# yurimjeon1892/EFGH

Measured on AMD Instinct MI355X. Metric: frame-pairs/sec EFGHNet fwd+bwd (384x1280 RGB + 64x2048 range), whole job, higher is better.
Workload: dtype f32; 1 GPU; BASELINE.json configs[2]: EFGHNet fwd+bwd with efghloss + gradient all-reduce + fused Adam, synthetic 384x1280 RGB + 131072-point sweep, batch=8 per GPU, random-init weights; global_batch=8, points=131072, parallelism=dp1

## Files before the change

efgh_amd/csrc/wgrad.hip:

```cpp
#include "common.h"

namespace {

typedef float f32x16 __attribute__((ext_vector_type(16)));
constexpr int TK = 128, TM = 32, LD = 128;

struct WArgs {
    const float *A; int64_t lda;
    int C, T, K;
    unsigned magicC;
    int Hin, Win, Hv, Wv, sh, sw;
    unsigned long long dhpack, dwpack;
    int Ho, Wo, osh, osw, oh0, ow0;
    const int *table;
    const float *G; int64_t ldg;
    int N;
    int tld;
    long long M; int mchunk;
    float *dW;
    long long zstride;
    unsigned kt, nt;
    long long bsA, bsG, bsD;
};

// ... 64 lines not shown
    }
    float4 rg[NGQ], ra[4];
    auto load_step = [&](long long ms) {
        if (TN != 128) {
#pragma unroll
            for (int q = 0; q < NGQ; ++q) {
                long long m = ms + gr0 + GRS * q;
                float4 g = make_float4(0.f, 0.f, 0.f, 0.f);
                if (m < mend && nin) g = *reinterpret_cast<const float4 *>(MODE == 1 ? git[q].g : p.G + m * p.ldg + n0 + gc4);
                rg[q] = g;
                if (MODE == 1) advance(git[q], n0 + gc4);
            }
        }
#pragma unroll
        for (int q = 0; q < 4; ++q) {
            long long m = ms + r0 + 8 * q;
            float4 g = make_float4(0.f, 0.f, 0.f, 0.f), a = g;
            if (m < mend) {
                if (MODE == 1) {
                    if (TN == 128 && nin) g = *reinterpret_cast<const float4 *>(rit[q].g);
                    if (kin && rit[q].rowok && (unsigned)(rit[q].j * p.sw + dw) < (unsigned)p.Win)
                        a = *reinterpret_cast<const float4 *>(rit[q].a);
                } else {
                    long long arow = -1;
                    if (MODE == 0) arow = m;
                    else if (kin) arow = p.table[m * (MODE == 4 ? p.tld : 16) + t];
                    if (TN == 128 && nin) g = *reinterpret_cast<const float4 *>(p.G + m * p.ldg + n0 + c4);
                    if (kin && arow >= 0) a = *reinterpret_cast<const float4 *>(p.A + arow * p.lda + c);
                }
            }
            if (TN == 128) rg[q] = g;
            ra[q] = a;
            if (MODE == 1) advance(rit[q], n0 + c4);
        }
    };

    f32x16 acc[2][TJ];
#pragma unroll
    for (int i = 0; i < 2; ++i)
#pragma unroll
        for (int j = 0; j < TJ; ++j)
#pragma unroll
            for (int r = 0; r < 16; ++r) acc[i][j][r] = 0.f;

    load_step(mbeg);
    for (long long ms = mbeg; ms < mend; ms += TM) {
#pragma unroll
        for (int q = 0; q < 4; ++q)
            *reinterpret_cast<float4 *>(&As[(r0 + 8 * q) * LD + c4]) = ra[q];
#pragma unroll
        for (int q = 0; q < NGQ; ++q)
            *reinterpret_cast<float4 *>(&Gs[(gr0 + GRS * q) * TN + gc4]) = rg[q];
        __syncthreads();
        if (ms + TM < mend) load_step(ms + TM);
#pragma unroll
        for (int mm = 0; mm < TM / 2; ++mm) {
            float g[2], a[TJ];
#pragma unroll
            for (int i = 0; i < 2; ++i) g[i] = Gs[(mm * 2 + lh) * TN + (wn * 2 + i) * 32 + l31];
#pragma unroll
            for (int j = 0; j < TJ; ++j) a[j] = As[(mm * 2 + lh) * LD + (wk * TJ + j) * 32 + l31];
#pragma unroll
            for (int i = 0; i < 2; ++i)
#pragma unroll
                for (int j = 0; j < TJ; ++j)
                    acc[i][j] = __builtin_amdgcn_mfma_f32_32x32x2f32(g[i], a[j], acc[i][j], 0, 0, 0);
        }
        __syncthreads();
    }
#pragma unroll
    for (int i = 0; i < 2; ++i)
#pragma unroll
        for (int j = 0; j < TJ; ++j) {
            const int k = k0 + (wk * TJ + j) * 32 + l31;
            if (k >= p.K) continue;
#pragma unroll
            for (int r = 0; r < 16; ++r) {
                const int n = n0 + (wn * 2 + i) * 32 + (r & 3) + 8 * (r >> 2) + 4 * lh;
                if (n < p.N) p.dW[(long long)n * p.K + k] = acc[i][j][r];
            }
        }
}

typedef efgh_wgrad_out_desc FoldUnpackArgs;

template <bool UNPACK>
__global__ void __launch_bounds__(256) k_fold_splits(const float4 *part, int zs, long long total4, float4 *dst, const FoldUnpackArgs u) {
    __shared__ float4 red[256];
    const int e = threadIdx.x & 15, zl = threadIdx.x >> 4;
    const long long i = (long long)blockIdx.x * 16 + e;
    float4 a = make_float4(0.f, 0.f, 0.f, 0.f), b = a;
    if (i < total4) {
        int z = zl;
        for (; z + 16 < zs; z += 32) {
            const float4 u = part[(long long)z * total4 + i], v = part[(long long)(z + 16) * total4 + i];
            a.x += u.x; a.y += u.y; a.z += u.z; a.w += u.w;
            b.x += v.x; b.y += v.y; b.z += v.z; b.w += v.w;
        }
        if (z < zs) { const float4 u = part[(long long)z * total4 + i]; a.x += u.x; a.y += u.y; a.z += u.z; a.w += u.w; }
        a.x += b.x; a.y += b.y; a.z += b.z; a.w += b.w;
    }
    red[threadIdx.x] = a;
    __syncthreads();
    for (int h = 8; h; h >>= 1) {
        if (zl < h) {
            const float4 o = red[threadIdx.x + h * 16];
            float4 m = red[threadIdx.x];
            m.x += o.x; m.y += o.y; m.z += o.z; m.w += o.w;
            red[threadIdx.x] = m;
        }
        __syncthreads();
    }
    if (zl == 0 && i < total4) {
        if (!UNPACK) { dst[i] = red[e]; return; }
        const float4 v4 = red[e];
        const float v[4] = {v4.x, v4.y, v4.z, v4.w};
        const long long idx = 4 * i;
        const int c0 = (int)(idx % u.Cp); const long long r = idx / u.Cp;
        const int t = (int)(r % u.T), n = (int)(r / u.T);
        if (n >= u.N) return;
        int ti = 0;
#pragma unroll
        for (int q = 0; q < 16; ++q) if (q == t) ti = u.taps[q];
#pragma unroll
        for (int q = 0; q < 4; ++q) {
            if (c0 + q >= u.C) continue;
            float *d = &u.W[n * u.sn + (c0 + q) * u.sc + ti * u.st];
            *d = u.accumulate ? *d + v[q] : v[q];
        }
    }
}

__global__ void k_unpack_weight(const float *__restrict__ Wp, float *__restrict__ W, int N, int T, int C,
                                int Cp, long long sn, long long sc, long long st, const int4 taps0,
                                const int4 taps1, const int4 taps2, const int4 taps3, int accumulate) {
    const int tp[16] = {taps0.x, taps0.y, taps0.z, taps0.w, taps1.x, taps1.y, taps1.z, taps1.w,
                        taps2.x, taps2.y, taps2.z, taps2.w, taps3.x, taps3.y, taps3.z, taps3.w};
    long long total = (long long)N * T * C;
    for (long long i = (long long)blockIdx.x * blockDim.x + threadIdx.x; i < total;
         i += (long long)gridDim.x * blockDim.x) {
        int c = (int)(i % C); long long r = i / C;
        int t = (int)(r % T); int n = (int)(r / T);
        int ti = 0;
#pragma unroll
        for (int q = 0; q < 16; ++q) if (q == t) ti = tp[q];
        float v = Wp[((long long)n * T + t) * Cp + c];
        float *dst = &W[n * sn + c * sc + ti * st];
        *dst = accumulate ? *dst + v : v;
    }
}

__global__ void __launch_bounds__(256)
k_table_scatter_add(const float *__restrict__ src, const int *__restrict__ table, long long M, int T, int C,
                    float *__restrict__ dst) {
    const int c4n = C >> 2;
    long long total = M * T * c4n;
    for (long long i = (long long)blockIdx.x * 256 + threadIdx.x; i < total; i += (long long)gridDim.x * 256) {
        int cq = (int)(i % c4n); long long r = i / c4n;
        int t = (int)(r % T); long long m = r / T;
        int row = table[m * 16 + t];
        if (row < 0) continue;
        float4 v = *reinterpret_cast<const float4 *>(src + (m * T + t) * C + cq * 4);
        float *d = dst + (long long)row * C + cq * 4;
        atomicAdd(d + 0, v.x); atomicAdd(d + 1, v.y); atomicAdd(d + 2, v.z); atomicAdd(d + 3, v.w);
    }
}

}

bool efgh_launch_fold_splits(const float *part, int zs, long long total, float *dst, hipStream_t st, const efgh_wgrad_out_desc *out) {
    const long long total4 = total / 4;
    const unsigned grid = (unsigned)((total4 + 15) / 16);
    if (out && out->W && out->T >= 1 && out->T <= 16 && out->Cp >= out->C && out->Cp % 4 == 0) {
        const long long row = (long long)out->T * out->Cp;
        if (total % row == 0 && total / row >= out->N && total / row < out->N + 4) {
            k_fold_splits<true><<<grid, 256, 0, st>>>((const float4 *)part, zs, total4, (float4 *)dst, *out);
            return true;
        }
    }
    FoldUnpackArgs none = {};
    k_fold_splits<false><<<grid, 256, 0, st>>>((const float4 *)part, zs, total4, (float4 *)dst, none);
    return false;
}

static int gather_wgrad_impl(const efgh_gemm_desc *d, const float *G, int64_t ldg, float *dWp, float *workspace, int nbatch,
                             int64_t bsG, int64_t bsD, const efgh_wgrad_out_desc *out, void *stream_, int tld = 0);


static long long wgrad_chunks(const efgh_gemm_desc *d, int nbatch, long long *chunk_out) {
    const int K = d->T * d->C;
    const int TN = d->N <= 64 ? 64 : 128;
    const long long kt = (K + TK - 1) / TK, nt = (d->N + TN - 1) / TN;
    static const int occ128[3] = {efgh_wg_per_cu((const void *)k_gather_wgrad<0, 128>, 256, 0), efgh_wg_per_cu((const void *)k_gather_wgrad<1, 128>, 256, 0),
                                  efgh_wg_per_cu((const void *)k_gather_wgrad<2, 128>, 256, 0)};
    static const int occ64[3] = {efgh_wg_per_cu((const void *)k_gather_wgrad<0, 64>, 256, 0), efgh_wg_per_cu((const void *)k_gather_wgrad<1, 64>, 256, 0),
                                 efgh_wg_per_cu((const void *)k_gather_wgrad<2, 64>, 256, 0)};
    const int mode = d->mode >= 0 && d->mode <= 2 ? d->mode : 0;
    return efgh_round_chunks(d->M, kt * nt * nbatch, TN == 128 ? occ128[mode] : occ64[mode], TM, 256, (double)nbatch * d->N * K, chunk_out);
}

extern "C" int64_t efgh_gather_wgrad_workspace(const efgh_gemm_desc *d) {
    if (!d || d->C <= 0 || d->T < 1 || d->N < 1 || d->M < 1) return 0;
    const int nbatch = d->nbatch > 1 ? d->nbatch : 1;
    const long long zs = wgrad_chunks(d, nbatch, nullptr);
    return zs > 1 ? zs * nbatch * (int64_t)d->N * d->T * d->C : 0;
}

extern "C" int efgh_gather_wgrad(const efgh_gemm_desc *d, const float *G, int64_t ldg, float *dWp, float *workspace,
                                 const efgh_wgrad_out_desc *out, void *stream_) {
    return gather_wgrad_impl(d, G, ldg, dWp, workspace, 1, 0, 0, out, stream_);
}

extern "C" int efgh_gather_wgrad_batched(const efgh_gemm_desc *d, const float *G, int64_t ldg, int64_t batch_stride_g,
                                         float *dWp, int64_t batch_stride_dw, float *workspace, void *stream_) {
    EFGH_CHECK_ARG(d && d->mode == 0 && d->nbatch >= 1 && d->nbatch <= 65535);
    EFGH_CHECK_ARG(d->batch_stride_a % 4 == 0 && batch_stride_g % 4 == 0 && batch_stride_dw == (int64_t)d->N * d->C);
    return gather_wgrad_impl(d, G, ldg, dWp, workspace, d->nbatch, batch_stride_g, batch_stride_dw, nullptr, stream_);
}

static int gather_wgrad_impl(const efgh_gemm_desc *d, const float *G, int64_t ldg, float *dWp, float *workspace, int nbatch,
                             int64_t bsG, int64_t bsD, const efgh_wgrad_out_desc *out, void *stream_, int tld) {
    hipStream_t st = (hipStream_t)stream_;
    EFGH_CHECK_ARG(d && d->A && G && dWp);
    EFGH_CHECK_ARG(d->C > 0 && d->C % 4 == 0 && d->T >= 1 && (d->T <= 16 || tld > 0) && d->N >= 1 && d->M >= 1);
    EFGH_CHECK_ARG(tld == 0 || (d->mode == 2 && d->table != nullptr && tld >= d->T && nbatch == 1 && !out));
    EFGH_CHECK_ARG(d->lda % 4 == 0 && ldg % 4 == 0 && d->N % 4 == 0);
    EFGH_CHECK_ARG((((uintptr_t)d->A) & 15) == 0 && (((uintptr_t)G) & 15) == 0 && (((uintptr_t)dWp) & 15) == 0);
    EFGH_CHECK_ARG((int64_t)d->T * d->C < 65536 && d->mode >= 0 && d->mode <= 2);
    WArgs a;
    a.A = d->A; a.lda = d->lda; a.C = d->C; a.T = d->T; a.K = d->T * d->C;
    a.magicC = (unsigned)((0x100000000ULL + d->C - 1) / d->C);
    a.Hin = d->Hin; a.Win = d->Win; a.Hv = d->Hv; a.Wv = d->Wv; a.sh = d->sh; a.sw = d->sw;
    a.dhpack = 0; a.dwpack = 0;
    for (int t = 0; t < 16; ++t) {
        int dh = t < d->T ? d->dh[t] : 0, dw = t < d->T ? d->dw[t] : 0;
        a.dhpack |= (unsigned long long)((dh + 8) & 15) << (4 * t);
        a.dwpack |= (unsigned long long)((dw + 8) & 15) << (4 * t);
    }
    a.Ho = d->Ho; a.Wo = d->Wo; a.osh = d->osh; a.osw = d->osw; a.oh0 = d->oh0; a.ow0 = d->ow0;
    a.table = d->table; a.G = G; a.ldg = ldg; a.N = d->N; a.M = d->M;
    a.bsA = nbatch > 1 ? d->batch_stride_a : 0; a.bsG = bsG; a.bsD = bsD; a.tld = tld;
    if (d->mode == 1) EFGH_CHECK_ARG(d->M == (int64_t)d->B * d->Hv * d->Wv && d->osh >= 1 && d->osw >= 1);
    if (d->mode == 2) EFGH_CHECK_ARG(d->table != nullptr);
    const int TN = a.N <= 64 ? 64 : 128;
    const int kt = (a.K + TK - 1) / TK, nt = (a.N + TN - 1) / TN;
    long long chunk = 0;
    const long long zs = wgrad_chunks(d, nbatch, &chunk);
    a.mchunk = (int)chunk;
    EFGH_CHECK_ARG(zs * kt * nt < 0x7fffffffLL);
    a.kt = (unsigned)kt; a.nt = (unsigned)nt;
    const long long plane = (long long)nbatch * a.N * a.K;
    EFGH_CHECK_ARG(zs == 1 || (workspace && (((uintptr_t)workspace) & 15) == 0));
    a.dW = zs > 1 ? workspace : dWp;
    a.zstride = zs > 1 ? plane : 0;
    const dim3 grid((unsigned)(zs * kt * nt), (unsigned)nbatch);
    if (tld > 0) {
        if (TN == 128) k_gather_wgrad<4, 128><<<grid, 256, 0, st>>>(a);
        else k_gather_wgrad<4, 64><<<grid, 256, 0, st>>>(a);
    } else if (TN == 128) {
        if (d->mode == 0) k_gather_wgrad<0, 128><<<grid, 256, 0, st>>>(a);
        else if (d->mode == 1) k_gather_wgrad<1, 128><<<grid, 256, 0, st>>>(a);
        else k_gather_wgrad<2, 128><<<grid, 256, 0, st>>>(a);
    } else {
        if (d->mode == 0) k_gather_wgrad<0, 64><<<grid, 256, 0, st>>>(a);
        else if (d->mode == 1) k_gather_wgrad<1, 64><<<grid, 256, 0, st>>>(a);
        else k_gather_wgrad<2, 64><<<grid, 256, 0, st>>>(a);
    }
    bool wrote = false;
    if (zs > 1) wrote = efgh_launch_fold_splits(workspace, (int)zs, plane, dWp, st, nbatch == 1 ? out : nullptr);
    EFGH_CHECK_LAUNCH();
    return wrote ? EFGH_WROTE_OUT : EFGH_OK;
}

extern "C" int efgh_blur_r_wgrad(const efgh_gemm_desc *d, int32_t ld, const float *G, int64_t ldg, float *dWp, float *workspace,
                                 void *stream_) {
    EFGH_CHECK_ARG(ld > 0);
    const int rc = gather_wgrad_impl(d, G, ldg, dWp, workspace, 1, 0, 0, nullptr, stream_, ld);
    return rc == EFGH_WROTE_OUT ? EFGH_OK : rc;
}

extern "C" int efgh_unpack_weight(const float *Wp, float *W, int32_t N, int32_t T, int32_t C, int32_t Cp,
                                  int64_t sn, int64_t sc, int64_t stt, const int32_t *tapidx, int32_t accumulate,
                                  void *stream_) {
    EFGH_CHECK_ARG(Wp && W && N > 0 && T > 0 && T <= 16 && C > 0 && Cp >= C);
    int tp[16];
    for (int t = 0; t < 16; ++t) tp[t] = (tapidx && t < T) ? tapidx[t] : (t < T ? t : 0);
    long long total = (long long)N * T * C;
    int grid = (int)((total + 255) / 256);
    if (grid > 8192) grid = 8192;
    k_unpack_weight<<<grid, 256, 0, (hipStream_t)stream_>>>(Wp, W, N, T, C, Cp, sn, sc, stt,
                                                           make_int4(tp[0], tp[1], tp[2], tp[3]),
                                                           make_int4(tp[4], tp[5], tp[6], tp[7]),
                                                           make_int4(tp[8], tp[9], tp[10], tp[11]),
                                                           make_int4(tp[12], tp[13], tp[14], tp[15]), accumulate);
    EFGH_CHECK_LAUNCH();
    return EFGH_OK;
}

extern "C" int efgh_table_scatter_add(const float *src, const int32_t *table, int64_t M, int32_t T, int32_t C,
                                      float *dst, void *stream_) {
    EFGH_CHECK_ARG(src && table && dst && M > 0 && T > 0 && T <= 16 && C % 4 == 0);
    long long total = M * T * (C / 4);
    long long g = (total + 255) / 256;
    k_table_scatter_add<<<(int)(g > 16384 ? 16384 : g), 256, 0, (hipStream_t)stream_>>>(src, table, M, T, C, dst);
    EFGH_CHECK_LAUNCH();
    return EFGH_OK;
}

extern "C" int efgh_debug_occupancy(char *out, int32_t cap) {
    EFGH_CHECK_ARG(out && cap > 64);
    snprintf(out, cap, "k_gather_wgrad<0,128> %d  <1,128> %d  <2,128> %d  <0,64> %d  <1,64> %d  <2,64> %d workgroups per CU",
             efgh_wg_per_cu((const void *)k_gather_wgrad<0, 128>, 256, 0), efgh_wg_per_cu((const void *)k_gather_wgrad<1, 128>, 256, 0),
             efgh_wg_per_cu((const void *)k_gather_wgrad<2, 128>, 256, 0), efgh_wg_per_cu((const void *)k_gather_wgrad<0, 64>, 256, 0),
             efgh_wg_per_cu((const void *)k_gather_wgrad<1, 64>, 256, 0), efgh_wg_per_cu((const void *)k_gather_wgrad<2, 64>, 256, 0));
    return EFGH_OK;
}
```

efgh_amd/ops.py:

```python
import ctypes
import os as _os
import threading
import weakref

import torch

from . import _C
from ._C import c_float, ptr

ACT_NONE, ACT_RELU, ACT_LEAKY = 0, 1, 2


def _L():
    return _C.lib()


def _st():
    return _C.stream_ptr()


def ceil4(n):
    return (n + 3) // 4 * 4


# ... 530 lines not shown

    def regroup():
        return Wp.view(N, S, Ts * C).permute(1, 0, 2).contiguous()
    Wg = _cached(Wp, ('ksplit', S), _ver(Wp), regroup)
    part = _scratch(S * M * N, dev)
    gather_gemm(A, lda, C, Ts, Wg, N, M, part, N, mode=2, table=table, a_off=a_off, batch=(S, 0, N * Ts * C, M * N, Ts),
                flops=flops if flops is not None else 2.0 * M * N * 15 * C, alias_mask=alias_mask)
    b = None
    if bias is not None:
        b = bias if bias.numel() == N else None
        assert b is not None
    _C.check(_L().efgh_fold_planes(ptr(part), S, M, N, ptr(b), act, slope, out.data_ptr() + 4 * out_off, ldo, _st()))


def gather_gemm(A, lda, C, T, Wp, N, M, out, ldo, mode=0, geom=None, table=None, bias=None, scale=None,
                shift=None, residual=None, ldr=0, act=ACT_NONE, slope=0.0, stats=None, a_off=0, out_off=0,
                res_off=0, M_dev=None, flops=None, batch=None, alias_mask=False, bn_bwd=None, pool=False, lazy=None, pre_v=None):
    key = (mode, C, N, T, geom, M, stats is not None, M_dev is not None, batch is not None, pool,
           scale is None and shift is None and residual is None and (bias is None or bias.numel() == N))
    route = gemm_route(*key)
    if (lazy is not None or pre_v is not None) and not (route == 'wino2d' and min(C, N) >= 64):
        raise _C.EfghError('gather_gemm(lazy= / pre_v=) on a launch the 2-D Winograd path does not serve (ask lazy_capable() first)')
    if route == 'blur_r':
        if (geom is not None or batch is not None or M_dev is not None or scale is not None or shift is not None or residual is not None
                or stats is not None or alias_mask or pool or bn_bwd is not None):
            raise _C.EfghError('gather_gemm(mode=MODE_BLUR_R) takes a plain blur launch: bias and activation only')
        blur_r_gemm(A, lda, C, T, Wp, N, M, out, ldo, table, bias=bias, act=act, slope=slope, a_off=a_off, out_off=out_off, flops=flops)
        return None
    if route == 'ksplit':
        return _blur_gemm_ksplit(A, lda, C, Wp, N, M, out, ldo, table, bias, act, slope, a_off, out_off, flops, alias_mask)
    d = _desc(A, lda, C, T, mode, N, M, geom, table, a_off, Wp, out, ldo, out_off, bias, scale, shift, residual, ldr, res_off, act, slope,
              stats, M_dev, batch)
    d.table_alias_mask = 1 if (alias_mask and mode == 2) else 0
    if route == 'sc' and not _sc_aligned(d, lda, ldo, residual, ldr, stats):
        route = gemm_route(*key, aligned=False)
    if pool and route not in ('c4', 'wino2d', 'wino_hpool'):
        raise _C.EfghError('gather_gemm(pool=True) on a launch no pooling epilogue serves (ask pool_fusable() first)')
    ev = _prof_start(PROFILE)
    bn_stats = None
    if route == 'thin':
        if TRACE_THIN is not None:
            TRACE_THIN.append(int(_L().efgh_thin_supported(ctypes.byref(d))))
        _C.check(_L().efgh_thin_gemm(ctypes.byref(d), _st()))
    elif route == 'c4':
        assert lda % 4 == 0
        _C.check((_L().efgh_c4_conv3x3_pooled if pool else _L().efgh_c4_conv3x3)(ctypes.byref(d), _st()))
    elif route == 'sc':
        _C.check(_L().efgh_sc_conv3x3(ctypes.byref(d), _st()))
    elif route == 'wino2d':
        if (bn_bwd is not None and stats is None and BN_BWD_FUSED_2D and out_off == 0 and not pool and bn_bwd.fits(M, N)
                and bn_bwd.y is None and bn_bwd.raw.stride(-2) % 4 == 0):
            rows = _L().efgh_wino2d_stats_rows(geom[0], geom[1], geom[2], N)
            bn_stats = _bn_bwd_sums(d, bn_bwd, rows, N, out.device)
        _wino2d_forward(d, A, a_off, lda, C, N, geom, Wp, pool=pool, lazy=lazy, pre_v=pre_v)
    elif route == 'wino_hpool':
        _C.check(_L().efgh_wino_conv3x3_hpool(ctypes.byref(d), ptr(wino_weight(Wp, N, C)), _st()))
    elif route == 'wino':
        if bn_bwd is not None and stats is None and BN_BWD_FUSED and out_off == 0 and bn_bwd.fits(M, N):
            rows = _L().efgh_wino_grid_m(geom[0], geom[1], geom[2])
            bn_stats = _bn_bwd_sums(d, bn_bwd, rows, N, out.device)
        _C.check(_L().efgh_wino_conv3x3(ctypes.byref(d), ptr(wino_weight(Wp, N, C)), _st()))
    else:
        _C.check(_L().efgh_gather_gemm(ctypes.byref(d), _st()))
    if ev is not None:
        _prof_end(ev, route, (mode, M, N, T, C), float(flops) if flops is not None else 2.0 * M * N * T * C, PROFILE, PROFILE_WINO,
                  batched=batch is not None)
    return bn_stats


def _bn_bwd_sums(d, src, rows, N, device):
    part = torch.empty((rows, 2, N), dtype=torch.float32, device=device)
    d.stats, d.stats_mode = part.data_ptr(), 1
    d.bn_raw, d.bn_ldraw = src.raw.data_ptr(), src.raw.stride(-2)
    if src.y is not None:
        d.bn_y, d.bn_ldy = src.y.data_ptr(), src.y.stride(-2)
    else:
        d.bn_pscale, d.bn_pshift = src.psc.data_ptr(), src.psh.data_ptr()
    d.bn_mean, d.bn_invstd = src.mean.data_ptr(), src.invstd.data_ptr()
    d.bn_act, d.bn_slope = src.act, src.slope
    return part


GEMM_DMA = True


def apply_switches():
    _L().efgh_gather_gemm_set_dma(1 if GEMM_DMA else 0)


PLANE_DMA = True
PLANE_DMA_NBUF = 0
PROFILE_WINO2D = None
PROFILE_WINO2D_GEMM = None
PLANES_SPLIT = None
PLANE_SPLIT_HITS = [0, 0]


def planes_split_active():
    if PLANES_SPLIT is not None:
        return bool(PLANES_SPLIT)
    return torch.backends.cuda.matmul.fp32_precision == 'tf32'


def _planes_split_now():
    m = TLS.planes_split
    return planes_split_active() if m is None else m


def _batched_plain_gemm(A3, W3, out3, rows, C, N):
    g = _desc(A3, 36 * C, C, 1, 0, N, rows, Wp=W3, out=out3, ldo=36 * N, batch=(36, C, N * C, N))
    ev = _prof_start(PROFILE_WINO2D_GEMM)
    if PLANE_DMA and _L().efgh_plane_gemm_supported(ctypes.byref(g)):
        if _planes_split_now():
            PLANE_SPLIT_HITS[0] += 1
            _C.check(_L().efgh_plane_gemm_x6(ctypes.byref(g), PLANE_DMA_NBUF, _st()))
        else:
            _C.check(_L().efgh_plane_gemm(ctypes.byref(g), PLANE_DMA_NBUF, _st()))
    else:
        _C.check(_L().efgh_gather_gemm(ctypes.byref(g), _st()))
    _prof_end(ev, 'planes', (0, rows, N, 36, C), 2.0 * 36 * rows * C * N, PROFILE_WINO2D_GEMM)


W2V_CACHE = {}
W2V_KEEP = True


def w2v_clear():
    me = threading.get_ident()
    with _LOCK:
        for k in [k for k, v in W2V_CACHE.items() if v[2] == me]:
            del W2V_CACHE[k]


POOL_FUSED = True
POOL_HALF = True


def pool_fusable(mode, C, N, geom, residual=None, stats=None):
    if not (POOL_FUSED and residual is None and stats is None and geom is not None and geom[1] >= 2 and geom[2] >= 2):
        return False
    route = gemm_route(mode, C, N, len(geom[7]), geom, geom[0] * geom[3] * geom[4], pool='h')
    if route == 'c4':
        return geom[5] == 1 and geom[6] == 1
    if route == 'wino2d':
        return True
    return 'h' if (route == 'wino_hpool' and POOL_HALF) else False


class LazyAct:
    __slots__ = ('scale', 'shift', 'act', 'slope')

    def __init__(self, scale, shift, act, slope):
        self.scale, self.shift, self.act, self.slope = scale, shift, act, slope


LAZY_ACT = True
W2_BWD_FUSED = True
W2_BWD_FUSED_POOL = True
LAZY_HITS = [0, 0]


def lazy_capable(mode, C, N, geom):
    return geom is not None and min(C, N) >= 64 and gemm_route(mode, C, N, len(geom[7]), geom, 0) == 'wino2d'


def wino2d_input(A, a_off, lda, C, B, H, W, V, lazy=None):
    if lazy is None:
        _C.check(_L().efgh_wino2d_input(A.data_ptr() + 4 * a_off, lda, C, B, H, W, ptr(V), _st()))
    else:
        LAZY_HITS[0] += 1
# ... 981 lines not shown
```

include/efgh_hip.h:

```cpp
#ifndef EFGH_HIP_H
#define EFGH_HIP_H
#include <stdint.h>

#ifdef __cplusplus
extern "C" {
#endif

#define EFGH_OK 0
#define EFGH_E_INVALID (-1)
#define EFGH_E_LAUNCH (-2)
#define EFGH_WROTE_OUT 1

const char *efgh_last_error(void);

#define EFGH_ABI_VERSION 4
int efgh_version(void);

#define EFGH_LATTICE_INFO_H 0
#define EFGH_LATTICE_INFO_ERR 1
#define EFGH_LATTICE_INFO_ALIAS 2
#define EFGH_LATTICE_INFO_CURSOR 3
#define EFGH_LATTICE_INFO_SEG 4
#define EFGH_LATTICE_MAX_SAMPLES 1024

// ... 269 lines not shown
    float bc2_sqrt;
    int32_t skip;
    int32_t nseg;
} efgh_guard_state;
int64_t efgh_grad_guard_workspace(int64_t n);
int efgh_grad_guard_measure(const float *g, int64_t n, const int64_t *bounds, int32_t nseg, double max_norm, float grad_scale,
                            int32_t skip_nonfinite, float beta1, float beta2, int32_t step, void *workspace,
                            efgh_guard_state *state, int32_t grid, void *stream);
int efgh_adam_step_guarded(float *w, const float *g, float *m, float *v, int64_t n, float lr, float beta1, float beta2,
                           float eps, float weight_decay, const efgh_guard_state *state, void *stream);

#define EFGH_ADAM_MAX_GROUPS 16
#define EFGH_ADAM_MAX_SEGMENTS 4096
typedef struct efgh_adam_groups {
    int32_t n_groups;
    int32_t step;
    float beta1, beta2, eps;
    float grad_scale;
    float lr[EFGH_ADAM_MAX_GROUPS];
    float weight_decay[EFGH_ADAM_MAX_GROUPS];
    float decay[EFGH_ADAM_MAX_GROUPS];
    int32_t decoupled[EFGH_ADAM_MAX_GROUPS];
} efgh_adam_groups;
int efgh_adam_step_groups(float *w, const float *g, float *m, float *v, int64_t n, const int64_t *seg_ends,
                          const uint8_t *seg_group, int32_t nseg, const int64_t *host_ends, const uint8_t *host_group,
                          const efgh_adam_groups *groups, const efgh_guard_state *state , int32_t grid,
                          void *stream);

int efgh_grad_drain(float *acc, float *g, int64_t n, int32_t first, void *stream);
int efgh_gimg_valid_count(const float *gdep4, const uint8_t *img_mask, int32_t B, int64_t HW, int64_t *count, void *stream);

typedef struct efgh_txn_state {
    int64_t forward_nonfinite;
    int64_t rolled_back;
    int64_t vetoed_total;
    int32_t first_bad;
    int32_t vetoed;
} efgh_txn_state;
int efgh_txn_snapshot(const float *live_f, float *shadow_f, int64_t nf, const int64_t *live_c, int64_t *shadow_c, int64_t nc,
                      efgh_txn_state *txn, void *stream);
int efgh_txn_probe(const float *live_f, const float *shadow_f, int64_t nf, const int64_t *starts, int32_t nseg, const float *losses,
                   int32_t k, int64_t loss_stride, efgh_txn_state *txn, void *stream);
int efgh_txn_resolve(float *live_f, const float *shadow_f, int64_t nf, int64_t *live_c, const int64_t *shadow_c, int64_t nc,
                     efgh_guard_state *guard, efgh_txn_state *txn, float beta1, float beta2, void *stream);

int efgh_ema_update(float *ema, const float *w, int64_t n, float decay, int32_t warmup, int64_t step,
                    const efgh_guard_state *state , void *stream);
int efgh_ema_swap(float *a, float *b, int64_t n, void *stream);

int efgh_thin_supported(const efgh_gemm_desc *d);
int efgh_thin_gemm(const efgh_gemm_desc *d, void *stream);
int64_t efgh_thin_wgrad_workspace(const efgh_gemm_desc *d);
int efgh_thin_wgrad(const efgh_gemm_desc *d, const float *G, int64_t ldg, float *dWp, float *workspace,
                    const efgh_wgrad_out_desc *out, void *stream);
int efgh_c4n4_supported(const efgh_gemm_desc *d);
int64_t efgh_c4n4_wgrad_workspace(const efgh_gemm_desc *d);
int efgh_c4n4_wgrad(const efgh_gemm_desc *d, const float *G, int64_t ldg, float *dWp, float *workspace,
                    const efgh_wgrad_out_desc *out, void *stream);

int efgh_sc_supported(const efgh_gemm_desc *d);
int32_t efgh_sc_stats_rows(int32_t B, int32_t H, int32_t W);
int efgh_sc_conv3x3(const efgh_gemm_desc *d, void *stream);
int efgh_sc_wgrad_supported(const efgh_gemm_desc *d);
int64_t efgh_sc_wgrad_workspace(const efgh_gemm_desc *d);
int efgh_sc_wgrad(const efgh_gemm_desc *d, const float *G, int64_t ldg, float *dWp, float *workspace,
                  const efgh_wgrad_out_desc *out, void *stream);
int efgh_c4_supported(const efgh_gemm_desc *d);
int32_t efgh_c4_stats_rows(int32_t B, int32_t Ho, int32_t Wo);
int efgh_c4_conv3x3(const efgh_gemm_desc *d, void *stream);
int efgh_c4_pooled_supported(const efgh_gemm_desc *d);
int efgh_c4_conv3x3_pooled(const efgh_gemm_desc *d, void *stream);
int efgh_c4_conv3x3_stats(const efgh_gemm_desc *d, void *stream);
int efgh_c4_conv3x3_pooled_train(const efgh_gemm_desc *d, const float *mean, const float *invstd, float *raw_win, void *stream);
int efgh_c4_pool_bwd_draw(const efgh_gemm_desc *d, const float *dy_pool, const float *mean, const float *invstd, const float *coef,
                          const double *m1, const double *m2, float *draw, void *stream);
int efgh_c4_wgrad_supported(const efgh_gemm_desc *d);
int64_t efgh_c4_wgrad_workspace(const efgh_gemm_desc *d);
int efgh_c4_wgrad(const efgh_gemm_desc *d, const float *G, int64_t ldg, float *dWp, float *workspace,
                  const efgh_wgrad_out_desc *out, void *stream);

int efgh_debug_occupancy(char *out, int32_t cap);

int efgh_gather_gemm_set_dma(int32_t on);

int efgh_plane_gemm_supported(const efgh_gemm_desc *d);
int efgh_plane_gemm(const efgh_gemm_desc *d, int32_t nbuf, void *stream);
int efgh_plane_wgrad_supported(const efgh_gemm_desc *d, int64_t ldg);
int64_t efgh_plane_wgrad_workspace(const efgh_gemm_desc *d);
int efgh_plane_wgrad_batched(const efgh_gemm_desc *d, const float *G, int64_t ldg, int64_t batch_stride_g, float *dWp,
                             int64_t batch_stride_dw, float *workspace, int32_t nbuf, void *stream);

int efgh_plane_gemm_x6(const efgh_gemm_desc *d, int32_t nbuf, void *stream);
int efgh_plane_wgrad_x6_batched(const efgh_gemm_desc *d, const float *G, int64_t ldg, int64_t batch_stride_g, float *dWp,
                                int64_t batch_stride_dw, float *workspace, int32_t nbuf, void *stream);

int efgh_convt_col2im(const float *Y, int64_t ldy, int32_t B, int32_t Hin, int32_t Win, int32_t Ho, int32_t Wo,
                      int32_t O, int32_t pad, const float *scale, const float *shift, int32_t act, float slope,
                      float *out, int64_t ldo, void *stream);
int efgh_convt_im2col(const float *G, int64_t ldg, int32_t B, int32_t Hin, int32_t Win, int32_t Ho, int32_t Wo,
                      int32_t O, int32_t pad, float *Ycol, int64_t ldy, void *stream);

int efgh_corr_pack_cam(const float *cam, const float *cam_mm, int32_t B, int32_t h, int32_t wc, int32_t segw,
                       int32_t nseg, int32_t nsplit, float *Wc, void *stream);
int efgh_corr_fold(const float *P, int32_t B, int32_t nsplit, int64_t Mv, int32_t ldp, int32_t nseg, int32_t segw,
                   int32_t nj, float *logit, float *score, void *stream);
int efgh_norm_bwd(const float *x, const float *dxn, const float *mm, int32_t B, int64_t n, float *part, float *dx, void *stream);
int efgh_corr_planes(const float *x, const float *mm, int32_t B, int32_t h, int32_t w, int32_t w_in_pitch, int32_t wP,
                     float *out, void *stream);
int efgh_corr_unplanes(const float *in, int32_t B, int32_t h, int32_t w, int32_t wP, float *out, void *stream);
int efgh_corr_toeplitz(const float *dl, int32_t B, int32_t nj, int32_t rows, int32_t cols, int32_t colsP, int32_t transpose,
                       float *T, void *stream);

int efgh_wino_supported(const efgh_gemm_desc *d);
int32_t efgh_wino_grid_m(int32_t B, int32_t H, int32_t W);
int efgh_wino_pack(const float *Wp, float *U, int32_t N, int32_t C, void *stream);
int efgh_wino_conv3x3_hpool(const efgh_gemm_desc *d, const float *U, void *stream);
int efgh_wino_conv3x3(const efgh_gemm_desc *d, const float *U, void *stream);
int efgh_wino_wgrad_supported(const efgh_gemm_desc *d);
int64_t efgh_wino_wgrad_workspace(const efgh_gemm_desc *d);
int efgh_wino_wgrad(const efgh_gemm_desc *d, const float *G, int64_t ldg, float *S, float *dWp, const efgh_wgrad_out_desc *out,
                    void *stream);

int efgh_prep_affine_nearest_u8(const uint8_t *in, int32_t h, int32_t w, const int64_t *coef6_host, uint8_t *out,
                                int32_t nh, int32_t nw, void *stream);
int efgh_prep_crop_pad_u8(const uint8_t *in, int32_t h, int32_t w, int32_t oy, int32_t ox, uint8_t *out, int32_t th,
                          int32_t tw, void *stream);
int efgh_prep_resample_u8(const uint8_t *in, int32_t h, int32_t w, int32_t axis, int32_t out_size, const int32_t *bounds,
                          const int32_t *coeffs, int32_t ksize, uint8_t *out, void *stream);
int efgh_prep_hwc_to_chw_u8(const uint8_t *in, int32_t h, int32_t w, uint8_t *chw, uint8_t *mask, void *stream);
int efgh_prep_u8_to_f32_chw_pad(const uint8_t *in, int32_t h, int32_t w, int32_t oy, int32_t ox, float *out, int32_t th,
                                int32_t tw, void *stream);
int32_t efgh_prep_filter_blocks(int32_t n);
int efgh_prep_radius_filter(const float *pcd, const int32_t *pre_idx, int32_t n, int32_t flip_xy, float radius,
                            int32_t *block_scratch, int32_t *keep_idx, int32_t *count, void *stream);
int efgh_prep_gather_transform(const float *pcd, const int32_t *keep_idx, const int32_t *sel, int32_t n_sel,
                               int32_t flip_xy, const double *T34, int32_t num_points, float *out32, double *out64,
                               void *stream);
int efgh_prep_sweeps_filter(const float *pts, int32_t stride, const int32_t *sweep_off, const double *M34,
                            const int32_t *identity, int32_t K, int32_t n_total, const int32_t *pre_idx, int32_t n,
                            int32_t flip_xy, double radius, float ego_x_half, float ego_y_half, int32_t *block_scratch,
                            int32_t *keep_idx, int32_t *count, void *stream);
int efgh_prep_sweeps_gather_transform(const float *pts, int32_t stride, const int32_t *sweep_off, const double *M34,
                                      const int32_t *identity, int32_t K, int32_t n_total, const int32_t *keep_idx,
                                      int32_t n_keep, const int32_t *sel, int32_t n_sel, int32_t flip_xy, const double *T34,
                                      int32_t num_points, float *out32, double *out64, void *stream);
int efgh_prep_sweeps_materialize(const float *pts, int32_t stride, const int32_t *sweep_off, const double *M34,
                                 const int32_t *identity, int32_t K, int32_t n_total, const int32_t *keep_idx, int32_t n,
                                 double *out, void *stream);
int64_t efgh_prep_voxel_workspace(int32_t n);
int efgh_prep_voxel_keep(const float *pts, int32_t stride, int32_t n_rows, const int32_t *keep_in, int32_t n_cap,
                         const int32_t *n_dev, double voxel, void *workspace, int32_t *keep_out, int32_t *count, void *stream);
int efgh_prep_sweeps_voxel_keep(const float *pts, int32_t stride, const int32_t *sweep_off, const double *M34,
                                const int32_t *identity, int32_t K, int32_t n_total, const int32_t *keep_in, int32_t n_cap,
                                const int32_t *n_dev, double voxel, void *workspace, int32_t *keep_out, int32_t *count,
                                void *stream);
#define EFGH_JITTER_MAX_OPS 4
#define EFGH_JITTER_BRIGHTNESS 0
#define EFGH_JITTER_CONTRAST 1
#define EFGH_JITTER_SATURATION 2
#define EFGH_JITTER_HUE 3
int32_t efgh_prep_jitter_partials(int64_t n_pixels);
int efgh_prep_jitter_sum(const uint8_t *in, int64_t n_pixels, const int32_t *ops_host, const float *factors_host, int32_t n_ops,
                         int32_t hue_shift, void *partials, void *stream);
int efgh_prep_jitter_apply(const uint8_t *in, int64_t n_pixels, const int32_t *ops_host, const float *factors_host, int32_t n_ops,
                           int32_t hue_shift, const void *partials, uint8_t *out, void *stream);

// ... 60 lines not shown
```

Measured before the change: 31.80 frame-pairs/s.

## Add async-DMA triple-buffered LDS ring kernel for gather weight-gradient GEMM

Adds a new weight-gradient kernel variant that streams the activation and output-gradient rows into a three-slot LDS ring via direct global-to-LDS 16-byte DMA. The next stages are prefetched while MFMA runs on the current one, and the kernel uses an XCD-aware block remapping. It is enabled by default for modes 0/1 when C is a multiple of 32, and split-K chunking is recomputed from the new kernel's occupancy. The aim is to hide global-load latency and cut register-staged copies, at the cost of larger dynamic LDS use, possibly lower occupancy, and a new code path with different store layout.

```diff
diff --git a/efgh_amd/csrc/wgrad.hip b/efgh_amd/csrc/wgrad.hip
--- a/efgh_amd/csrc/wgrad.hip
+++ b/efgh_amd/csrc/wgrad.hip
@@ -170,6 +170,172 @@
         }
 }
 
+__device__ __attribute__((aligned(512))) float g_wgrad_zero[128];
+constexpr int WD_TS = 16, WD_NSLOT = 3;
+
+template <int MODE, int TN>
+__global__ void __launch_bounds__(256, TN == 128 ? 3 : 4)
+k_gather_wgrad_dma(const WArgs p0) {
+    static_assert(MODE == 0 || MODE == 1, "plain rows or an image geometry");
+    constexpr int TJ = TN == 128 ? 2 : 1;
+    constexpr int TS = WD_TS;
+    constexpr int NAP = 2;
+    constexpr int NGP = TN == 128 ? 2 : 1;
+    constexpr int GRP = TN == 128 ? 2 : 4;
+    constexpr int SLOT = TS * (TN + LD);
+    extern __shared__ __attribute__((aligned(1024))) float ring[];
+    WArgs p = p0;
+    p.A += (long long)blockIdx.y * p0.bsA; p.G += (long long)blockIdx.y * p0.bsG; p.dW += (long long)blockIdx.y * p0.bsD;
+    const int tid = threadIdx.x, lane = tid & 63, wave = __builtin_amdgcn_readfirstlane(tid >> 6);
+    const int wn = TN == 128 ? (wave >> 1) : 0, wk = TN == 128 ? (wave & 1) : wave;
+    const int l31 = lane & 31, lh = lane >> 5;
+    const unsigned ring_lds = lds_addr(ring);
+    const unsigned nblk = gridDim.x, q8 = nblk >> 3, r8 = nblk & 7, xcd = blockIdx.x & 7, within = blockIdx.x >> 3;
+    const unsigned lin = (xcd < r8 ? xcd * (q8 + 1) : r8 * (q8 + 1) + (xcd - r8) * q8) + within;
+    const unsigned per_z = p.kt * p.nt, bz = lin / per_z, rem = lin - bz * per_z;
+    const unsigned by = rem / p.kt, bx = rem - by * p.kt;
+    const int k0 = bx * TK, n0 = by * TN;
+    const long long mbeg = (long long)bz * p.mchunk;
+    long long mend = mbeg + p.mchunk;
+    if (mend > p.M) mend = p.M;
+    if (mbeg >= mend) return;
+    p.dW += (long long)bz * p.zstride;
+
+    const int ar0 = wave * 4 + lh, c4 = l31 * 4;
+    const int gr0 = wave * 4 + (TN == 128 ? lh : lane >> 4);
+    const int gcol = n0 + (TN == 128 ? c4 : (lane & 15) * 4);
+    const int kk = k0 + c4;
+    const bool kin = kk < p.K, nin = gcol < p.N;
+    const int t = (int)(((unsigned long long)kk * p.magicC) >> 32);
+    const int c = kk - t * p.C;
+    const int dh = (int)((p.dhpack >> (4 * (t & 15))) & 15) - 8, dw = (int)((p.dwpack >> (4 * (t & 15))) & 15) - 8;
+    const float *zsrc = g_wgrad_zero + c4;
+
+    struct RowIt { int j, i; long long b; const float *g, *a; bool rowok; };
+    auto point = [&](RowIt &it) {
+        const long long orow = (it.b * p.Ho + (it.i * p.osh + p.oh0)) * p.Wo + (it.j * p.osw + p.ow0);
+        it.g = p.G + orow * p.ldg + gcol;
+        const int ih = it.i * p.sh + dh;
+        it.rowok = (unsigned)ih < (unsigned)p.Hin;
+        it.a = p.A + ((it.b * p.Hin + ih) * p.Win + (it.j * p.sw + dw)) * p.lda + c;
+    };
+    auto place = [&](RowIt &it, long long m) {
+        if (MODE == 0) { it.g = p.G + m * p.ldg + gcol; it.a = p.A + m * p.lda + c; it.rowok = true; it.j = it.i = 0; it.b = 0; return; }
+        it.j = (int)(m % p.Wv); const long long r = m / p.Wv;
+        it.i = (int)(r % p.Hv); it.b = r / p.Hv;
+        point(it);
+    };
+    const long long gstep = (long long)TS * (MODE == 1 ? p.osw : 1) * p.ldg, astep = (long long)TS * (MODE == 1 ? p.sw : 1) * p.lda;
+    const bool narrow = p.Wv < 4 * TM;
+    auto advance = [&](RowIt &it) {
+        it.g += gstep; it.a += astep;
+        if (MODE == 0) return;
+        it.j += TS;
+        if (narrow || it.j >= p.Wv) {
+            while (it.j >= p.Wv) { it.j -= p.Wv; ++it.i; }
+            while (it.i >= p.Hv) { it.i -= p.Hv; ++it.b; }
+            point(it);
+        }
+    };
+    RowIt rit[NAP], git[NGP];
+#pragma unroll
+    for (int q = 0; q < NAP; ++q) place(rit[q], mbeg + ar0 + 2 * q);
+    if (TN != 128) {
+#pragma unroll
+        for (int q = 0; q < NGP; ++q) place(git[q], mbeg + gr0 + GRP * q);
+    }
+    auto issue = [&](long long ms, int buf) {
+        const unsigned base = ring_lds + (unsigned)(buf * SLOT) * 4u;
+#pragma unroll
+        for (int q = 0; q < NGP; ++q) {
+            RowIt &it = TN == 128 ? rit[q] : git[q];
+            const bool ok = ms + gr0 + GRP * q < mend && nin;
+            dma16(ok ? it.g : zsrc, base + (unsigned)(wave * NGP + q) * 1024u);
+            if (TN != 128) advance(it);
+        }
+#pragma unroll
+        for (int q = 0; q < NAP; ++q) {
+            bool ok = ms + ar0 + 2 * q < mend && kin && rit[q].rowok;
+            if (MODE == 1) ok = ok && (unsigned)(rit[q].j * p.sw + dw) < (unsigned)p.Win;
+            dma16(ok ? rit[q].a : zsrc, base + (unsigned)(TS * TN) * 4u + (unsigned)(wave * NAP + q) * 1024u);
+            advance(rit[q]);
+        }
+    };
+
+    f32x16 acc[2][TJ];
+#pragma unroll
+    for (int i = 0; i < 2; ++i)
+#pragma unroll
+        for (int j = 0; j < TJ; ++j)
+#pragma unroll
+            for (int r = 0; r < 16; ++r) acc[i][j][r] = 0.f;
+
+    const int nst = (int)((mend - mbeg + TS - 1) / TS);
+    issue(mbeg, 0);
+    if (nst > 1) issue(mbeg + TS, 1);
+    const int gx = lh * TN + wn * 64 + 2 * l31;
+    const int ax = TS * TN + lh * LD + (TN == 128 ? wk * 64 + 2 * l31 : wk * 32 + l31);
+    int cur = 0;
+    for (int s = 0; s < nst; ++s) {
+        if (s + 1 < nst) wait_vm<NAP + NGP>();
+        else wait_vm<0>();
+        __builtin_amdgcn_s_barrier();
+        asm volatile("" ::: "memory");
+        const int nxt = cur == 0 ? WD_NSLOT - 1 : cur - 1;
+        if (s + 2 < nst) issue(mbeg + (long long)(s + 2) * TS, nxt);
+        const float *Gs = ring + cur * SLOT;
+        cur = cur + 1 == WD_NSLOT ? 0 : cur + 1;
+        if constexpr (TN == 128) {
+            float2 g[2], a[2];
+            g[0] = *reinterpret_cast<const float2 *>(Gs + gx);
+            a[0] = *reinterpret_cast<const float2 *>(Gs + ax);
+#pragma unroll
+            for (int mm = 0; mm < TS / 2; ++mm) {
+                if (mm + 1 < TS / 2) {
+                    g[(mm + 1) & 1] = *reinterpret_cast<const float2 *>(Gs + (mm + 1) * 2 * TN + gx);
+                    a[(mm + 1) & 1] = *reinterpret_cast<const float2 *>(Gs + (mm + 1) * 2 * LD + ax);
+                }
+                __builtin_amdgcn_sched_barrier(0);
+                const float2 cg = g[mm & 1], ca = a[mm & 1];
+                acc[0][0] = __builtin_amdgcn_mfma_f32_32x32x2f32(cg.x, ca.x, acc[0][0], 0, 0, 0);
+                acc[0][1] = __builtin_amdgcn_mfma_f32_32x32x2f32(cg.x, ca.y, acc[0][1], 0, 0, 0);
+                acc[1][0] = __builtin_amdgcn_mfma_f32_32x32x2f32(cg.y, ca.x, acc[1][0], 0, 0, 0);
+                acc[1][1] = __builtin_amdgcn_mfma_f32_32x32x2f32(cg.y, ca.y, acc[1][1], 0, 0, 0);
+                __builtin_amdgcn_sched_barrier(0);
+            }
+        } else {
+            float2 g[2]; float a[2];
+            g[0] = *reinterpret_cast<const float2 *>(Gs + gx);
+            a[0] = Gs[ax];
+#pragma unroll
+            for (int mm = 0; mm < TS / 2; ++mm) {
+                if (mm + 1 < TS / 2) {
+                    g[(mm + 1) & 1] = *reinterpret_cast<const float2 *>(Gs + (mm + 1) * 2 * TN + gx);
+                    a[(mm + 1) & 1] = Gs[(mm + 1) * 2 * LD + ax];
+                }
+                __builtin_amdgcn_sched_barrier(0);
+                const float2 cg = g[mm & 1]; const float ca = a[mm & 1];
+                acc[0][0] = __builtin_amdgcn_mfma_f32_32x32x2f32(cg.x, ca, acc[0][0], 0, 0, 0);
+                acc[1][0] = __builtin_amdgcn_mfma_f32_32x32x2f32(cg.y, ca, acc[1][0], 0, 0, 0);
+                __builtin_amdgcn_sched_barrier(0);
+            }
+        }
+    }
+    const int kb = k0 + (TN == 128 ? wk * 64 + 2 * l31 : wk * 32 + l31);
+    if (kb >= p.K) return;
+#pragma unroll
+    for (int q = 0; q < 2; ++q) {
+#pragma unroll
+        for (int r = 0; r < 16; ++r) {
+            const int n = n0 + wn * 64 + 2 * ((r & 3) + 8 * (r >> 2) + 4 * lh) + q;
+            if (n >= p.N) continue;
+            float *dp = p.dW + (long long)n * p.K + kb;
+            if constexpr (TN == 128) *reinterpret_cast<float2 *>(dp) = make_float2(acc[q][0][r], acc[q][1][r]);
+            else *dp = acc[q][0][r];
+        }
+    }
+}
+
 typedef efgh_wgrad_out_desc FoldUnpackArgs;
 
 template <bool UNPACK>
@@ -275,7 +441,16 @@
                              int64_t bsG, int64_t bsD, const efgh_wgrad_out_desc *out, void *stream_, int tld = 0);
 
 
-static long long wgrad_chunks(const efgh_gemm_desc *d, int nbatch, long long *chunk_out) {
+std::atomic<unsigned long long> g_wdma_raised[4];
+static bool g_wgrad_dma = true;
+static std::atomic<long long> g_wgrad_census[2];
+
+static bool wgrad_dma_ok(const efgh_gemm_desc *d, int tld) {
+    return g_wgrad_dma && tld == 0 && (d->mode == 0 || d->mode == 1) && d->C % 32 == 0;
+}
+static constexpr size_t wgrad_dma_lds(int TN) { return (size_t)WD_NSLOT * WD_TS * (TN + LD) * sizeof(float); }
+
+static long long wgrad_chunks(const efgh_gemm_desc *d, int nbatch, bool dma, long long *chunk_out) {
     const int K = d->T * d->C;
     const int TN = d->N <= 64 ? 64 : 128;
     const long long kt = (K + TK - 1) / TK, nt = (d->N + TN - 1) / TN;
@@ -283,14 +458,19 @@
                                   efgh_wg_per_cu((const void *)k_gather_wgrad<2, 128>, 256, 0)};
     static const int occ64[3] = {efgh_wg_per_cu((const void *)k_gather_wgrad<0, 64>, 256, 0), efgh_wg_per_cu((const void *)k_gather_wgrad<1, 64>, 256, 0),
                                  efgh_wg_per_cu((const void *)k_gather_wgrad<2, 64>, 256, 0)};
+    static const int occdma128[2] = {efgh_wg_per_cu((const void *)k_gather_wgrad_dma<0, 128>, 256, wgrad_dma_lds(128)),
+                                     efgh_wg_per_cu((const void *)k_gather_wgrad_dma<1, 128>, 256, wgrad_dma_lds(128))};
+    static const int occdma64[2] = {efgh_wg_per_cu((const void *)k_gather_wgrad_dma<0, 64>, 256, wgrad_dma_lds(64)),
+                                    efgh_wg_per_cu((const void *)k_gather_wgrad_dma<1, 64>, 256, wgrad_dma_lds(64))};
     const int mode = d->mode >= 0 && d->mode <= 2 ? d->mode : 0;
-    return efgh_round_chunks(d->M, kt * nt * nbatch, TN == 128 ? occ128[mode] : occ64[mode], TM, 256, (double)nbatch * d->N * K, chunk_out);
+    const int occ = dma ? (TN == 128 ? occdma128[mode] : occdma64[mode]) : (TN == 128 ? occ128[mode] : occ64[mode]);
+    return efgh_round_chunks(d->M, kt * nt * nbatch, occ, TM, 256, (double)nbatch * d->N * K, chunk_out);
 }
 
 extern "C" int64_t efgh_gather_wgrad_workspace(const efgh_gemm_desc *d) {
     if (!d || d->C <= 0 || d->T < 1 || d->N < 1 || d->M < 1) return 0;
     const int nbatch = d->nbatch > 1 ? d->nbatch : 1;
-    const long long zs = wgrad_chunks(d, nbatch, nullptr);
+    const long long zs = wgrad_chunks(d, nbatch, wgrad_dma_ok(d, 0), nullptr);
     return zs > 1 ? zs * nbatch * (int64_t)d->N * d->T * d->C : 0;
 }
 
@@ -304,6 +484,16 @@
     EFGH_CHECK_ARG(d && d->mode == 0 && d->nbatch >= 1 && d->nbatch <= 65535);
     EFGH_CHECK_ARG(d->batch_stride_a % 4 == 0 && batch_stride_g % 4 == 0 && batch_stride_dw == (int64_t)d->N * d->C);
     return gather_wgrad_impl(d, G, ldg, dWp, workspace, d->nbatch, batch_stride_g, batch_stride_dw, nullptr, stream_);
+}
+
+template <int MODE, int TN>
+static int launch_wgrad_dma(const WArgs &a, const dim3 &grid, hipStream_t st) {
+    if (!efgh_raise_lds_once(g_wdma_raised[MODE * 2 + (TN == 128)], (const void *)k_gather_wgrad_dma<MODE, TN>, (int)wgrad_dma_lds(TN))) {
+        efgh_set_error("%s:%d: cannot raise the dynamic LDS limit of k_gather_wgrad_dma", __FILE__, __LINE__);
+        return EFGH_E_LAUNCH;
+    }
+    k_gather_wgrad_dma<MODE, TN><<<grid, 256, wgrad_dma_lds(TN), st>>>(a);
+    return EFGH_OK;
 }
 
 static int gather_wgrad_impl(const efgh_gemm_desc *d, const float *G, int64_t ldg, float *dWp, float *workspace, int nbatch,
@@ -333,7 +523,8 @@
     const int TN = a.N <= 64 ? 64 : 128;
     const int kt = (a.K + TK - 1) / TK, nt = (a.N + TN - 1) / TN;
     long long chunk = 0;
-    const long long zs = wgrad_chunks(d, nbatch, &chunk);
+    const bool dma = wgrad_dma_ok(d, tld);
+    const long long zs = wgrad_chunks(d, nbatch, dma, &chunk);
     a.mchunk = (int)chunk;
     EFGH_CHECK_ARG(zs * kt * nt < 0x7fffffffLL);
     a.kt = (unsigned)kt; a.nt = (unsigned)nt;
@@ -342,7 +533,13 @@
     a.dW = zs > 1 ? workspace : dWp;
     a.zstride = zs > 1 ? plane : 0;
     const dim3 grid((unsigned)(zs * kt * nt), (unsigned)nbatch);
-    if (tld > 0) {
+    g_wgrad_census[dma ? 1 : 0].fetch_add(1, std::memory_order_relaxed);
+    if (dma) {
+        int rc;
+        if (TN == 128) rc = d->mode == 0 ? launch_wgrad_dma<0, 128>(a, grid, st) : launch_wgrad_dma<1, 128>(a, grid, st);
+        else rc = d->mode == 0 ? launch_wgrad_dma<0, 64>(a, grid, st) : launch_wgrad_dma<1, 64>(a, grid, st);
+        if (rc != EFGH_OK) return rc;
+    } else if (tld > 0) {
         if (TN == 128) k_gather_wgrad<4, 128><<<grid, 256, 0, st>>>(a);
         else k_gather_wgrad<4, 64><<<grid, 256, 0, st>>>(a);
     } else if (TN == 128) {
@@ -358,6 +555,24 @@
     if (zs > 1) wrote = efgh_launch_fold_splits(workspace, (int)zs, plane, dWp, st, nbatch == 1 ? out : nullptr);
     EFGH_CHECK_LAUNCH();
     return wrote ? EFGH_WROTE_OUT : EFGH_OK;
+}
+
+extern "C" int efgh_gather_wgrad_set_dma(int32_t on) {
+    const int old = g_wgrad_dma ? 1 : 0;
+    g_wgrad_dma = on != 0;
+    return old;
+}
+
+extern "C" int efgh_gather_wgrad_census(int64_t *count) {
+    EFGH_CHECK_ARG(count);
+    count[0] = g_wgrad_census[0].load(std::memory_order_relaxed);
+    count[1] = g_wgrad_census[1].load(std::memory_order_relaxed);
+    return EFGH_OK;
+}
+
+extern "C" int64_t efgh_gather_wgrad_chunks(const efgh_gemm_desc *d) {
+    if (!d || d->C <= 0 || d->T < 1 || d->N < 1 || d->M < 1) return 0;
+    return wgrad_chunks(d, d->nbatch > 1 ? d->nbatch : 1, wgrad_dma_ok(d, 0), nullptr);
 }
 
 extern "C" int efgh_blur_r_wgrad(const efgh_gemm_desc *d, int32_t ld, const float *G, int64_t ldg, float *dWp, float *workspace,
@@ -397,9 +612,14 @@
 
 extern "C" int efgh_debug_occupancy(char *out, int32_t cap) {
     EFGH_CHECK_ARG(out && cap > 64);
-    snprintf(out, cap, "k_gather_wgrad<0,128> %d  <1,128> %d  <2,128> %d  <0,64> %d  <1,64> %d  <2,64> %d workgroups per CU",
+    snprintf(out, cap, "k_gather_wgrad<0,128> %d  <1,128> %d  <2,128> %d  <0,64> %d  <1,64> %d  <2,64> %d  "
+             "k_gather_wgrad_dma<0,128> %d  <1,128> %d  <0,64> %d  <1,64> %d workgroups per CU",
              efgh_wg_per_cu((const void *)k_gather_wgrad<0, 128>, 256, 0), efgh_wg_per_cu((const void *)k_gather_wgrad<1, 128>, 256, 0),
              efgh_wg_per_cu((const void *)k_gather_wgrad<2, 128>, 256, 0), efgh_wg_per_cu((const void *)k_gather_wgrad<0, 64>, 256, 0),
-             efgh_wg_per_cu((const void *)k_gather_wgrad<1, 64>, 256, 0), efgh_wg_per_cu((const void *)k_gather_wgrad<2, 64>, 256, 0));
+             efgh_wg_per_cu((const void *)k_gather_wgrad<1, 64>, 256, 0), efgh_wg_per_cu((const void *)k_gather_wgrad<2, 64>, 256, 0),
+             efgh_wg_per_cu((const void *)k_gather_wgrad_dma<0, 128>, 256, wgrad_dma_lds(128)),
+             efgh_wg_per_cu((const void *)k_gather_wgrad_dma<1, 128>, 256, wgrad_dma_lds(128)),
+             efgh_wg_per_cu((const void *)k_gather_wgrad_dma<0, 64>, 256, wgrad_dma_lds(64)),
+             efgh_wg_per_cu((const void *)k_gather_wgrad_dma<1, 64>, 256, wgrad_dma_lds(64)));
     return EFGH_OK;
 }
diff --git a/efgh_amd/ops.py b/efgh_amd/ops.py
--- a/efgh_amd/ops.py
+++ b/efgh_amd/ops.py
@@ -636,10 +636,12 @@
 
 
 GEMM_DMA = True
+WGRAD_DMA = True
 
 
 def apply_switches():
     _L().efgh_gather_gemm_set_dma(1 if GEMM_DMA else 0)
+    _L().efgh_gather_wgrad_set_dma(1 if WGRAD_DMA else 0)
 
 
 PLANE_DMA = True
diff --git a/include/efgh_hip.h b/include/efgh_hip.h
--- a/include/efgh_hip.h
+++ b/include/efgh_hip.h
@@ -375,6 +375,9 @@
 int efgh_debug_occupancy(char *out, int32_t cap);
 
 int efgh_gather_gemm_set_dma(int32_t on);
+int efgh_gather_wgrad_set_dma(int32_t on);
+int efgh_gather_wgrad_census(int64_t *count);
+int64_t efgh_gather_wgrad_chunks(const efgh_gemm_desc *d);
 
 int efgh_plane_gemm_supported(const efgh_gemm_desc *d);
 int efgh_plane_gemm(const efgh_gemm_desc *d, int32_t nbuf, void *stream);
```

Result: no change. 32.10 frame-pairs/s (median of 6 runs) (+1.0%).
